# Aqasch/TensorRL-QAS

Measured on AMD Instinct MI355X. Metric: VQE env-steps/sec, higher is better.
Workload: dtype f64

## Files before the change

### tensorrl-qas_amd/csrc/vqe_device.h

```cpp
#pragma once
#include <hip/hip_runtime.h>
#include <stdint.h>
#ifdef VQE_STAMPS
__device__ unsigned long long g_cby_dbg[8];
__device__ unsigned long long g_cby_in_out[2];
__device__ long long g_cby_t0_unused;
#if defined(__HIP_DEVICE_COMPILE__)
#define CBY_STAMP_RESET() long long cby_t0_ = (long long)__builtin_readcyclecounter(); (void)cby_t0_
#define CBY_STAMP(k)                                                                               \
  {                                                                                                \
    const long long t_ = (long long)__builtin_readcyclecounter();                                  \
    if (ctx.tid == 0 && Ctx::nth > 1) __hip_atomic_fetch_add(&g_cby_dbg[k], (unsigned long long)(t_ - cby_t0_), __ATOMIC_RELAXED, __HIP_MEMORY_SCOPE_AGENT); \
    cby_t0_ = (long long)__builtin_readcyclecounter();                                             \
  }
#else
#define CBY_STAMP_RESET()
#define CBY_STAMP(k)
#endif
#endif
#include "cobyla_m0.h"
#include "vqe_geo.h"

namespace vqe {

// ... 451 lines not shown
            L.ops[nops] = Op{xm[r.q0], zm[r.q0], r.pidx, r.kind | (int)(((c >> r.q0) & 1u) << 8)};
          ++nops;
          break;
        default: break;
      }
    }
    int permuted = (c != 0);
    for (int q = 0; q < n; ++q) if (xm[q] != (1u << q)) permuted = 1;
    L.meta[0] = nops < A.max_ops ? nops : A.max_ops;
    L.meta[1] = (int32_t)c;
    L.meta[2] = phase;
    L.meta[3] = permuted;
    L.meta[6] = permuted;
    L.meta[7] = (int32_t)c;
  }
  __syncthreads();
}

template <int N>
__device__ __forceinline__ void patch_noise_wave(const BatchArgs& A, int b, uint64_t eval_id, const Lds& L, int skip,
                                                 bool canonical, int lane, int skip_end) {
  const int G = A.gate_count[b];
  const int4* gsrc = (const int4*)(A.gates + A.gate_begin[b]);
  {
    Op* exe = N >= 10 ? L.sched : L.ops;
    const int kmax = L.meta[0];
    const uint64_t lt_mask = lane ? (~0ull >> (64 - lane)) : 0ull;
    const uint64_t nkey = noise_key(A.noise.seed, (uint64_t)b, eval_id);
    uint32_t c = 0;
    int ny = 0, kbase = 0;
    int4 rnext = lane < G ? gsrc[lane] : make_int4(-1, 0, 0, 0);
    for (int base = 0; base < G; base += 64) {
      const int i = base + lane;
      int kind = -1, q0 = 0, q1 = 0, code = 0;
      const int4 r = rnext;
      if (i + 64 < G) rnext = gsrc[i + 64];
      if (i < G && !(i >= skip && i < skip_end)) {
        kind = r.x; q0 = r.y; q1 = r.z < 0 ? 0 : r.z;
        if (kind == G_DEPOL1 || kind == G_DEPOL2) {
          const double u = noise_uniform_k(nkey, (uint64_t)(i - ((skip >= 0 && i >= skip_end) ? skip_end - skip : 0)));
          if (kind == G_DEPOL1) { if (u < A.noise.p1) code = 1 + (int)(u / A.noise.p1 * 3.0); }
          else if (u < A.noise.p2) code = 1 + (int)(u / A.noise.p2 * 15.0);
        }
      }
      const int pa = kind == G_DEPOL1 ? code : (kind == G_DEPOL2 ? (code & 3) : 0);
      const int pb = kind == G_DEPOL2 ? (code >> 2) : 0;
      const uint32_t flip_a = (pa == 1 || pa == 2) ? 1u << q0 : 0u;
      const uint32_t flip_b = (pb == 1 || pb == 2) ? 1u << q1 : 0u;
      const uint32_t cnot_m = kind == G_CNOT ? 1u << q1 : 0u;
      const int nrec = (kind >= G_RX && kind <= G_DEPOL1) ? 1 : (kind == G_DEPOL2 ? 2 : 0);
      const uint32_t w1 = flip_a | ((uint32_t)q0 << 16) | ((uint32_t)q1 << 24);
      const uint32_t w2 = cnot_m | (flip_b << 16);
      const uint64_t has1 = __ballot(nrec >= 1), has2 = __ballot(nrec == 2);
      const int k0 = kbase + __popcll(has1 & lt_mask) + __popcll(has2 & lt_mask);
      kbase += __popcll(has1) + __popcll(has2);
      ny += __popcll(__ballot(pa == 2)) + __popcll(__ballot(pb == 2));
      uint64_t inv0 = 0, inv1 = 0;
      const int cnt = G - base < 64 ? G - base : 64;
      int j0 = 0;
      if (c == 0) {
        const uint64_t flips = __ballot((flip_a | flip_b) != 0u);
        j0 = flips ? __ffsll((long long)flips) - 1 : cnt;
      }
      for (int j = j0; j < cnt; ++j) {
        const uint32_t a = (uint32_t)__builtin_amdgcn_readlane((int)w1, j);
        const uint32_t bw = (uint32_t)__builtin_amdgcn_readlane((int)w2, j);
        c ^= a & 0xffffu;
        const uint32_t b0 = (c >> ((a >> 16) & 31u)) & 1u;
        c ^= (0u - b0) & (bw & 0xffffu);
        inv0 |= (uint64_t)b0 << j;
        c ^= bw >> 16;
        inv1 |= (uint64_t)((c >> (a >> 24)) & 1u) << j;
      }
      auto apply = [&](int pk, int sign, int pauli) {
        if (pk < kmax) {
          Op* o = exe + L.sidx[pk];
          int kd = o->kind;
          if (pauli >= 0) kd = (kd & ~0xff) | ((pauli == 2 || pauli == 3) ? OP_PZ : OP_NOP);
          o->kind = (kd & ~0x100) | (sign << 8);
        }
      };
      if (nrec >= 1) apply(k0, (int)((inv0 >> lane) & 1ull), kind <= G_RZ ? -1 : pa);
      if (nrec == 2) apply(k0 + 1, (int)((inv1 >> lane) & 1ull), pb);
    }
    {
      const int ns = N >= 10 ? L.meta[4] : kmax;
      int lead = 0;
      for (int base = ((ns - 1) / 64) * 64; base >= 0; base -= 64) {
        const int k = base + lane;
        const int kd = k < ns ? exe[k].kind : 0;
        const bool nop = k < ns && (kd & 0xff) == OP_NOP;
        const uint64_t m = __ballot(nop);
        const uint64_t behind = lane < 63 ? (m >> (lane + 1)) : 0ull;
        const int in_chunk = 63 - lane;
        int run = behind == ~0ull >> (lane + 1) && lane < 63 ? in_chunk : (lane < 63 ? __ffsll((long long)~behind) - 1 : 0);
        if (run >= in_chunk) run = in_chunk + lead;
        if (k < ns) exe[k].kind = (kd & 0x00ffffff) | ((run < 255 ? run : 255) << 24);
        lead = (m == ~0ull) ? 64 + lead : __ffsll((long long)~m) - 1;
      }
    }
    if (lane == 0) {
      uint32_t cs = c;
      if (N >= 10 && canonical) {
        cs = 0;
        for (int q = 0; q < N; ++q) cs |= (uint32_t)parity32(A.ham.mrow[q] & c) << q;
      }
      L.meta[1] = (int32_t)cs;
      L.meta[2] = (3 * ny) & 3;
      L.meta[3] = L.meta[6] | (c != 0);
      L.meta[7] = (int32_t)c;
    }
  }
}

template <int N>
__device__ __forceinline__ void patch_noise(const BatchArgs& A, int b, uint64_t eval_id, const Lds& L, int skip,
                                            bool canonical, int skip_end = 0) {
  if (threadIdx.x < 64) patch_noise_wave<N>(A, b, eval_id, L, skip, canonical, (int)threadIdx.x, skip_end);
  __syncthreads();
}

}
#include "vqe_reg.h"
namespace vqe {

template <int N>
__device__ __forceinline__ void compile_all(const BatchArgs& A, int b, uint64_t eval_id, const Lds& L, int skip = -1,
                                            bool canonical = true, bool slots = false, int skip_end = 0) {
  compile_ops(A, b, eval_id, L, skip, slots, skip_end);
  if constexpr (N < 10) {
    if (slots) {
      for (int k = threadIdx.x; k < L.meta[0]; k += (int)blockDim.x) L.sidx[k] = (uint16_t)k;
      __syncthreads();
    }
  }
  if constexpr (N >= kRegMinQubits) {
    if (threadIdx.x == 0) schedule_ops<N>(L);
    __syncthreads();
    if (canonical) {
      uint32_t zrow = 0, cbit = 0;
      if (threadIdx.x < N) {
        const uint32_t m = A.ham.mrow[threadIdx.x];
        for (int q = 0; q < N; ++q) if ((m >> q) & 1u) zrow ^= L.zm[q];
        cbit = (uint32_t)parity32(m & (uint32_t)L.meta[1]) << threadIdx.x;
      }
      uint32_t cnew = cbit;
#pragma unroll
      for (int o = 8; o > 0; o >>= 1) cnew |= __shfl_xor(cnew, o, 16);
      __syncthreads();
      if (threadIdx.x < N) L.zm[threadIdx.x] = zrow;
      if (threadIdx.x == 0) L.meta[1] = (int32_t)cnew;
      __syncthreads();
    }
  }
}

template <int N, bool SLOTS = true>
__device__ __forceinline__ void run_ops(const Lds& L, const double* theta, int P, int p_hole = -1) {
  constexpr int kThreads = Geo<N>::NT;
  constexpr uint32_t DIM = 1u << N;
  constexpr int NP = (DIM / 2 + kThreads - 1) / kThreads;
  constexpr int NA = (DIM + kThreads - 1) / kThreads;
  const int tid = threadIdx.x;
  for (int j = tid; j < P; j += kThreads) {
    if (j == p_hole) continue;
    double s, c;
    sincos(0.5 * theta[j - (p_hole >= 0 && j > p_hole)], &s, &c);
    L.cs[j] = make_double2(c, s);
  }
  __syncthreads();
  const int nops = L.meta[0];
  for (int o = 0; o < nops; ++o) {
    const Op op = L.ops[o];
    const int kind = op.kind & 0xff;
    if constexpr (SLOTS) o += (int)((uint32_t)op.kind >> 24);
    if (kind == OP_NOP) continue;
    const int inv = (op.kind >> 8) & 1;
    if (kind == OP_RX || kind == OP_RY) {
      const double2 cs = L.cs[op.pidx];
      const int hb = 31 - __clz((int)op.xm);
      if (kind == OP_RX) {
#pragma unroll
        for (int k = 0; k < NP; ++k) {
          const uint32_t q = tid + k * kThreads;
          if (DIM / 2 >= kThreads || q < DIM / 2) {
            const uint32_t p0 = insert0(q, hb), p1 = p0 ^ op.xm;
            const double2 a0 = L.psi[p0], a1 = L.psi[p1];
            L.psi[p0] = make_double2(cs.x * a0.x - cs.y * a1.y, cs.x * a0.y + cs.y * a1.x);
            L.psi[p1] = make_double2(cs.x * a1.x - cs.y * a0.y, cs.x * a1.y + cs.y * a0.x);
          }
        }
      } else {
#pragma unroll
        for (int k = 0; k < NP; ++k) {
          const uint32_t q = tid + k * kThreads;
          if (DIM / 2 >= kThreads || q < DIM / 2) {
            const uint32_t p0 = insert0(q, hb), p1 = p0 ^ op.xm;
            const double s0 = (parity32(p0 & op.zm) ^ inv) ? -cs.y : cs.y;
            const double2 a0 = L.psi[p0], a1 = L.psi[p1];
            L.psi[p0] = make_double2(cs.x * a0.x + s0 * a1.x, cs.x * a0.y + s0 * a1.y);
            L.psi[p1] = make_double2(cs.x * a1.x - s0 * a0.x, cs.x * a1.y - s0 * a0.y);
          }
        }
      }
    } else if (kind == OP_RZ) {
      const double2 cs = L.cs[op.pidx];
#pragma unroll
      for (int k = 0; k < NA; ++k) {
        const uint32_t p = tid + k * kThreads;
        if (DIM >= kThreads || p < DIM) {
          const double s = (parity32(p & op.zm) ^ inv) ? -cs.y : cs.y;
          const double2 a = L.psi[p];
          L.psi[p] = make_double2(cs.x * a.x - s * a.y, cs.x * a.y + s * a.x);
        }
      }
    } else if (kind == OP_PZ) {
#pragma unroll
      for (int k = 0; k < NA; ++k) {
        const uint32_t p = tid + k * kThreads;
        if ((DIM >= kThreads || p < DIM) && (parity32(p & op.zm) ^ inv)) {
          const double2 a = L.psi[p];
          L.psi[p] = make_double2(-a.x, -a.y);
        }
      }
    }
    __syncthreads();
  }
  if (L.meta[3]) {
    const uint32_t c = (uint32_t)L.meta[1];
    double2 tmp[NA];
#pragma unroll
    for (int k = 0; k < NA; ++k) {
      const uint32_t i = tid + k * kThreads;
      if (DIM >= kThreads || i < DIM) {
        uint32_t v = i ^ c, p = 0;
#pragma unroll
        for (int q = 0; q < N; ++q) p ^= ((v >> q) & 1u) ? L.xm[q] : 0u;
        tmp[k] = L.psi[p];
      }
    }
    __syncthreads();
#pragma unroll
    for (int k = 0; k < NA; ++k) {
      const uint32_t i = tid + k * kThreads;
      if (DIM >= kThreads || i < DIM) L.psi[i] = tmp[k];
    }
    __syncthreads();
  }
}

template <int N>
__device__ __forceinline__ void load_init(const Lds& L, const double2* init) {
  constexpr int kThreads = Geo<N>::NT;
  constexpr uint32_t DIM = 1u << N;
  constexpr int NA = (DIM + kThreads - 1) / kThreads;
#pragma unroll
  for (int k = 0; k < NA; ++k) {
    const uint32_t p = threadIdx.x + k * kThreads;
    if (DIM >= kThreads || p < DIM) L.psi[p] = init[p];
  }
}


constexpr int kEnergyBatch = 4;

#define VQE_ENERGY_PAIRS(X, HB, DEXPR)                                                             \
  {                                                                                                \
    const uint32_t base = insert0(tid, (HB)) << 4, basex = base ^ ((X) << 4);                     \
    uint32_t kbit[KB > 0 ? KB : 1];                                                                \
    _Pragma("unroll") for (int i = 0; i < KB; ++i)                                                \
      kbit[i] = 16u << (LT + i + ((LT + i) >= (HB) ? 1 : 0));                                     \
    double p0s = 0.0, p1s = 0.0;                                                                   \
    _Pragma("unroll") for (int k0 = 0; k0 < NP; k0 += kEnergyBatch) {                             \
      constexpr int NB = NP < kEnergyBatch ? NP : kEnergyBatch;                                   \
      double2 pa[NB], pb[NB];                                                                      \
      _Pragma("unroll") for (int kk = 0; kk < NB; ++kk) {                                         \
        const int k = k0 + kk;                                                                     \
        uint32_t kc = 0;                                                                           \
        _Pragma("unroll") for (int i = 0; i < KB; ++i) if ((k >> i) & 1) kc ^= kbit[i];           \
        const bool live = FULL || tid + (uint32_t)k * kThreads < DIM / 2;                         \
        pb[kk] = live ? *(const double2*)(psi_b + (base ^ kc)) : make_double2(0.0, 0.0);         \
        pa[kk] = live ? *(const double2*)(psi_b + (basex ^ kc)) : make_double2(0.0, 0.0);        \
      }                                                                                            \
      __builtin_amdgcn_sched_barrier(0);                                                           \
      _Pragma("unroll") for (int kk = 0; kk < NB; ++kk) {                                         \
        const int k = k0 + kk;                                                                     \
        const double v = (pa[kk].x * pb[kk].x + pa[kk].y * pb[kk].y) * (DEXPR);                   \
        if (k & 1) p1s += v; else p0s += v;                                                       \
      }                                                                                            \
    }                                                                                              \
    acc0 += p0s;                                                         \
    acc1 += p1s;                                                                                   \
  }

#define VQE_ENERGY_CONSUME(G, D)                                                                   \
  {                                                                                                \
    const GroupMeta m = L.gm[G];                                                                   \
    const uint32_t x = (uint32_t)__builtin_amdgcn_readfirstlane((int)m.x);                        \
    const int hb = __builtin_amdgcn_readfirstlane(m.hb);                                          \
    VQE_ENERGY_PAIRS(x, hb, D[k])                                                                  \
  }

template <int N>
__device__ __forceinline__ void energy_real_lds(const Lds& L, const double* __restrict__ tables, int g0, int g1,
                                                double& acc0, double& acc1) {
  constexpr int kThreads = Geo<N>::NT;
// ... 524 lines not shown
        first += kStage * kThreads;
      }
    }
    for (int i0 = first; i0 < nw; i0 += kStage * kThreads) {
      double2 v[kStage];
#pragma unroll
      for (int k = 0; k < kStage; ++k) {
        const int i = i0 + k * kThreads;
        v[k] = s[i < nw ? i : nw - 1];
      }
#pragma unroll
      for (int k = 0; k < kStage; ++k) asm volatile("" : "+v"(v[k].x), "+v"(v[k].y));
#pragma unroll
      for (int k = 0; k < kStage; ++k) {
        const int i = i0 + k * kThreads;
        if (i < nw) d[i] = v[k];
      }
    }
    __syncthreads();
  }
  __device__ __forceinline__ bool out(bool full = true, double2* cs_out = nullptr, int P = 0, int p_hole = -1) {
    if (threadIdx.x == 0) { pub[0] = want; pub[1] = nfvals; }
    __syncthreads();
    want = pub[0]; nfvals = pub[1];
    if (!staged || resident) return false;
    const bool light = VQE_LIGHT_OUT && !full && want && cs_out != nullptr;
    if (light) {
      for (int j = threadIdx.x; j < P; j += kThreads) {
        if (j == p_hole) continue;
        double sn, cn;
        sincos(0.5 * lmem[j - (p_hole >= 0 && j > p_hole)], &sn, &cn);
        cs_out[j] = make_double2(cn, sn);
      }
    }
    const double2* s = (const double2*)lmem;
    double2* d = (double2*)gmem;
    const int nw = (words + 1) / 2;
    for (int i0 = threadIdx.x; i0 < nw; i0 += kStage * kThreads) {
      double2 v[kStage];
#pragma unroll
      for (int k = 0; k < kStage; ++k) {
        const int i = i0 + k * kThreads;
        v[k] = s[i < nw ? i : nw - 1];
      }
#pragma unroll
      for (int k = 0; k < kStage; ++k) asm volatile("" : "+v"(v[k].x), "+v"(v[k].y));
#pragma unroll
      for (int k = 0; k < kStage; ++k) {
        const int i = i0 + k * kThreads;
        if (i < nw) d[i] = v[k];
      }
    }
    if (light) {
      asm volatile("s_waitcnt lgkmcnt(0)\n\ts_barrier" ::: "memory");
      return true;
    }
    __syncthreads();
    return false;
  }
  template <bool FIRST, class Cob, class Ptr>
  __device__ __forceinline__ void call(Ptr mem, double f, double rhobeg, double rhoend, int maxfun) {
    Cob cob;
    cob.ctx.tid = Cob::P == 0 ? 0 : (int)(threadIdx.x % (unsigned)decltype(cob.ctx)::nth);
    if constexpr (!std::is_base_of<WaveCtx, decltype(cob.ctx)>::value) cob.ctx.red = red;
    if constexpr (decltype(cob.ctx)::kTile) {
      if constexpr (std::is_base_of<WaveCtx, decltype(cob.ctx)>::value) {
        cob.ctx.tile = (lds_double*)tile;
        cob.ctx.shared = (lds_double*)tile + Cob::kTileDoubles;
      } else {
        cob.ctx.tile = (lds_double*)lmem + (threadIdx.x >> 6) * Cob::kTileDoubles;
        cob.ctx.shared = (lds_double*)lmem + (kThreads / 64) * Cob::kTileDoubles;
      }
    }
    int nn = n;
    if constexpr (N >= 10) asm volatile("" : "+s"(mem), "+s"(nn));
    cob.bind(mem, nn);
    if (FIRST) {
      want = cob.start(rhobeg, rhoend, maxfun);
    } else {
      cob.load_state();
      want = cob.tell(f);
    }
    nfvals = cob.nfvals;
    cob.save_state();
  }
  bool cs_ready;
  template <bool FIRST, class Side>
  __device__ __forceinline__ int run(double f, double rhobeg, double rhoend, int maxfun, Side side, bool full = true,
                                     double2* cs_out = nullptr, int P = 0, int p_hole = -1) {
#ifdef VQE_STAMPS
    const long long t0 = clock64();
#endif
    in();
#ifdef VQE_STAMPS
    const long long t1 = clock64();
#endif
    if (kBlock && block) {
      if constexpr (kBlock) {
        if (kThreads == 64 || (threadIdx.x >= 64 && threadIdx.x < 128)) side();
        call<FIRST, CobB>(gmem, f, rhobeg, rhoend, maxfun);
      }
    } else if (threadIdx.x < 64) {
      if (staged) call<FIRST, CobL>((lds_double*)lmem, f, rhobeg, rhoend, maxfun);
      else if (rows_ctx()) {
        if constexpr (kRowsG) call<FIRST, CobR>(gmem, f, rhobeg, rhoend, maxfun);
      } else call<FIRST, CobG>(gmem, f, rhobeg, rhoend, maxfun);
      if constexpr (kThreads == 64) side();
    } else if (threadIdx.x < 128) {
#ifdef VQE_STAMPS
      const long long ts0 = clock64();
#endif
      side();
#ifdef VQE_STAMPS
      if (threadIdx.x == 64 && !FIRST) atomicAdd(&g_cby_dbg[6], (unsigned long long)(clock64() - ts0));
#endif
    }
#ifdef VQE_STAMPS
    const long long t2 = clock64();
#endif
    cs_ready = out(full, cs_out, P, p_hole);
#ifdef VQE_STAMPS
    if (threadIdx.x == 0 && !FIRST) {
      atomicAdd(&g_cby_dbg[7], (unsigned long long)(t2 - t1));
      atomicAdd(&g_cby_in_out[0], (unsigned long long)(t1 - t0));
      atomicAdd(&g_cby_in_out[1], (unsigned long long)(clock64() - t2));
    }
#endif
    return want;
  }
  __device__ __forceinline__ int start(double rhobeg, double rhoend, int maxfun, bool full = true, double2* cs_out = nullptr,
                                       int P = 0, int p_hole = -1) {
    return run<true>(0.0, rhobeg, rhoend, maxfun, NoSide(), full, cs_out, P, p_hole);
  }
  template <class Side>
  __device__ __forceinline__ int tell(double f, unsigned long long* __restrict__ dbg, Side side, bool full = true,
                                      double2* cs_out = nullptr, int P = 0, int p_hole = -1) {
#ifdef VQE_STAMPS
    const long long t0 = clock64();
#endif
    const int w = run<false>(f, 0.0, 0.0, 0, side, full, cs_out, P, p_hole);
#ifdef VQE_STAMPS
    if (threadIdx.x == 0) atomicAdd(dbg + 4, (unsigned long long)(clock64() - t0));
#endif
    return w;
  }
};

template <int N>
__global__ void __launch_bounds__(Geo<N>::NT) k_lds_energy(BatchArgs A) {
  extern __shared__ __attribute__((aligned(16))) unsigned char smem[];
  const Lds L = carve(smem, N, A.max_ops, A.max_params, A.ham.n_groups, A.max_pair);
  const int b = blockIdx.x;
  const bool noisy = (A.noise.p1 > 0.0 || A.noise.p2 > 0.0);
  stage_groups(A.ham, L);
  if constexpr (N >= 10) stage_cls<N>(A.ham, L);
  compile_all<N>(A, b, 0, L, -1, true, noisy);
  if (noisy) patch_noise<N>(A, b, A.noise.eval_base, L, -1, true);
  double e = lds_evaluate<N, true>(A, L, A.theta + A.par_begin[b], A.par_count[b]);
  if (A.noise.shot_sigma != 0.0) e += A.noise.shot_sigma * noise_gauss(A.noise.seed, (uint64_t)b, A.noise.eval_base);
  if (threadIdx.x == 0) { A.fout[b] = e; if (A.nfev) A.nfev[b] = 1; }
}

template <int N>
__global__ void __launch_bounds__(Geo<N>::NT) k_lds_state(BatchArgs A) {
  constexpr int kThreads = Geo<N>::NT;
  extern __shared__ __attribute__((aligned(16))) unsigned char smem[];
  const Lds L = carve(smem, N, A.max_ops, A.max_params, A.ham.n_groups, A.max_pair);
  const bool noisy_state = (A.noise.p1 > 0.0 || A.noise.p2 > 0.0);
  compile_all<N>(A, 0, 0, L, -1, false, noisy_state);
  if (noisy_state) patch_noise<N>(A, 0, A.noise.eval_base, L, -1, false);
  if constexpr (N >= kRegMinQubits) {
    run_ops_reg<N, true>(L, A.init, A.theta + A.par_begin[0], A.par_count[0]);
  } else {
    load_init<N>(L, A.init);
    __syncthreads();
    run_ops<N>(L, A.theta + A.par_begin[0], A.par_count[0]);
  }
  const int ph = L.meta[2];
  for (uint32_t p = threadIdx.x; p < (1u << N); p += kThreads) {
    double2 a = L.psi[p];
    if (ph == 1) a = make_double2(-a.y, a.x);
    else if (ph == 2) a = make_double2(-a.x, -a.y);
    else if (ph == 3) a = make_double2(a.y, -a.x);
    A.state_out[p] = a;
  }
}

template <int N, bool WIDE = (N >= 10 && Geo<N>::NT >= 256), bool NOISY = false>
__global__ void __launch_bounds__(Geo<N>::NT, Geo<N>::WPS) k_lds_minimize(BatchArgs A) {
  constexpr int kThreads = Geo<N>::NT;
  extern __shared__ __attribute__((aligned(16))) unsigned char smem[];
  const Lds L = carve(smem, N, A.max_ops, A.max_params, A.ham.n_groups, A.max_pair);
  const int b = A.order[blockIdx.x];
  const int P = A.par_count[b];
  const double* theta = A.theta + A.par_begin[b];
  double* xout = A.xout + A.par_begin[b];
  constexpr bool noisy = NOISY;
  const int skip = A.new_gate ? A.new_gate[b] : -1;
  int p_hole = -1;
  int skip_end = skip + 1;
  if (skip >= 0) {
    const GateRec r = A.gates[A.gate_begin[b] + skip];
    if (r.kind >= G_RX && r.kind <= G_RZ) p_hole = r.pidx;
    if (skip + 1 < A.gate_count[b]) {
      const GateRec f = A.gates[A.gate_begin[b] + skip + 1];
      if ((f.kind == G_DEPOL1 && r.kind >= G_RX && r.kind <= G_RZ && f.q0 == r.q0) ||
          (f.kind == G_DEPOL2 && r.kind == G_CNOT && f.q0 == r.q0 && f.q1 == r.q1))
        skip_end = skip + 2;
    }
  }
  const int Popt = P - (p_hole >= 0);
  stage_groups(A.ham, L);
  if constexpr (N >= 10) stage_cls<N>(A.ham, L);
  StagedCobyla<N, WIDE> sc;
  sc.cs_ready = false;
  const bool full_out = N < 10 || A.trace != nullptr;
  int phase = 0, nfev = 1;
  bool need_compile = true;
  bool patched = false;
  double fret = 0.0, flast = 0.0;
  if (Popt > 0) {
    sc.init(A.scratch + A.scratch_begin[b], L, Popt);
    for (int j = threadIdx.x; j < P; j += kThreads)
      if (j != p_hole) sc.x()[j - (p_hole >= 0 && j > p_hole)] = theta[j];
    __syncthreads();
    sc.start(A.rhobeg, A.rhoend, A.maxfun, full_out, L.cs, P, p_hole);
    phase = 1;
  }
  for (;;) {
    const double* th = phase == 0 ? theta : (phase == 1 ? sc.x() : xout);
    const int sk = phase == 2 ? -1 : skip;
    const int ske = phase == 2 ? 0 : skip_end;
    const int ph = phase == 2 ? -1 : p_hole;
    const uint64_t eid = A.noise.eval_base +
                         (phase == 1 ? (uint64_t)sc.nfvals : (phase == 2 ? (uint64_t)A.maxfun + 1 : 0));
    if (need_compile) { compile_all<N>(A, b, 0, L, sk, true, noisy, ske); need_compile = false; patched = false; }
    if (noisy && !patched) patch_noise<N>(A, b, eid, L, sk, true, ske);
    patched = false;
    const bool csr = phase == 1 && sc.cs_ready;
    double e = lds_evaluate<N, NOISY>(A, L, th, P, ph, [&]() { if (phase == 1) sc.prefetch(); }, csr);
    if (A.noise.shot_sigma != 0.0) e += A.noise.shot_sigma * noise_gauss(A.noise.seed, (uint64_t)b, eid);
    bool finished_opt = false;
    if (phase == 0) {
      fret = e;
      for (int j = threadIdx.x; j < P; j += kThreads) {
        xout[j] = A.env_step ? (double)(float)theta[j] : theta[j];
        A.xraw[A.par_begin[b] + j] = theta[j];
      }
      finished_opt = true;
    } else if (phase == 1) {
      flast = e;
      if (A.trace) {
        double* tr = A.trace + ((size_t)b * A.maxfun + (size_t)(sc.nfvals - 1)) * (size_t)(1 + A.max_params);
        if (threadIdx.x == 0) tr[0] = e;
        for (int j = threadIdx.x; j < Popt; j += kThreads) tr[1 + j] = sc.x()[j];
      }
#ifdef VQE_STAMPS
      const long long tt0 = clock64();
#endif
      const uint64_t eid_next = A.noise.eval_base + (uint64_t)sc.nfvals + 1;
      const int want = sc.tell(e, A.dbg, [&]() {
        if (noisy) patch_noise_wave<N>(A, b, eid_next, L, sk, true, (int)(threadIdx.x & 63), ske);
      }, full_out, L.cs, P, p_hole);
      patched = noisy && want;
#ifdef VQE_STAMPS
      if (threadIdx.x == 0) atomicAdd(A.dbg + 3, (unsigned long long)(clock64() - tt0));
#endif
      if (!want) {
        for (int j = threadIdx.x; j < P; j += kThreads) {
          const double v = (j == p_hole) ? theta[j] : sc.x()[j - (p_hole >= 0 && j > p_hole)];
          xout[j] = A.env_step ? (double)(float)v : v;
          A.xraw[A.par_begin[b] + j] = v;
        }
        const double* st = sc.state();
        fret = ((int)st[11] == cby::DONE_RHOEND && (int)st[10] == 1) ? flast : st[4];
        nfev = sc.nfvals;
        finished_opt = true;
      }
    } else {
      fret = e;
      break;
    }
    if (finished_opt) {
      if (!A.env_step) break;
      __syncthreads();
      phase = 2;
      need_compile = true;
    }
  }
  if (threadIdx.x == 0) { A.fout[b] = fret; A.nfev[b] = nfev; }
}

}
```

### tensorrl-qas_amd/csrc/vqe_reg.h

```cpp
#pragma once
#include "vqe_geo.h"

namespace vqe {

enum : int { OP_RELAYOUT = 5 };

struct LayoutRec {
  uint32_t e[5];
  uint32_t pos;
  uint32_t pos8;
  uint32_t pad;
};

struct Basis {
  uint32_t* e;
  int32_t* piv;
  int k;
  __device__ void clear() { k = 0; }
  __device__ uint32_t reduce(uint32_t v) const {
    for (int i = 0; i < k; ++i) if ((v >> piv[i]) & 1u) v ^= e[i];
    return v;
  }
  __device__ bool add(uint32_t v) {
    v = reduce(v);
    if (!v) return false;
    const int p = 31 - __clz((int)v);
    for (int i = 0; i < k; ++i) if ((e[i] >> p) & 1u) e[i] ^= v;
    e[k] = v; piv[k] = p; ++k;
    return true;
  }
  __device__ uint32_t coords(uint32_t v) const {
    uint32_t j = 0;
    for (int i = 0; i < k; ++i) j |= ((v >> piv[i]) & 1u) << i;
    return j;
  }
};

template <int N>
__device__ __forceinline__ void emit_layout(const Basis& B, LayoutRec* out) {
  uint32_t pivmask = 0;
  for (int i = 0; i < 5; ++i) out->e[i] = i < B.k ? B.e[i] : 0u;
  for (int i = 0; i < B.k; ++i) pivmask |= 1u << B.piv[i];
  uint32_t pos = 0, pos8 = 0;
  int cnt = 0;
  for (int b = 0; b < N; ++b)
    if (!((pivmask >> b) & 1u)) {
      if (cnt < 8) pos |= (uint32_t)b << (4 * cnt); else pos8 = (uint32_t)b;
      ++cnt;
    }
  out->pos = pos;
  out->pos8 = pos8;
}

template <int R>
__device__ __forceinline__ uint32_t sign_word(uint32_t svec) {
  constexpr uint32_t pat[5] = {0xAAAAAAAAu, 0xCCCCCCCCu, 0xF0F0F0F0u, 0xFF00FF00u, 0xFFFF0000u};
  uint32_t w = 0;
#pragma unroll
  for (int i = 0; i < R; ++i) if ((svec >> i) & 1u) w ^= pat[i];
  return w;
}

template <int N>
__device__ __forceinline__ void schedule_ops(const Lds& L) {
  constexpr int R = N - Geo<N>::LT;
  const int nraw = L.meta[0];
  int ns = 0, nl = 0;
  Basis B;
  B.e = (uint32_t*)L.sb;
  B.piv = (int32_t*)L.sb + 8;
  auto open_layout = [&](int from) {
    B.clear();
    for (int k = from; k < nraw && B.k < R; ++k) {
      const int kd = L.ops[k].kind & 0xff;
      if (kd == OP_RX || kd == OP_RY) B.add(L.ops[k].xm);
    }
    for (int b = N - 1; b >= 0 && B.k < R; --b) B.add(1u << b);
    emit_layout<N>(B, &L.lay[nl]);
    ++nl;
  };
  open_layout(0);
  for (int o = 0; o < nraw; ++o) {
    const Op op = L.ops[o];
    const int kd = op.kind & 0xff;
    uint32_t j = 0;
    if (kd == OP_RX || kd == OP_RY) {
      if (B.reduce(op.xm) != 0) {
        open_layout(o);
        L.sched[ns++] = Op{(uint32_t)(nl - 1), 0u, -1, OP_RELAYOUT};
      }
      j = B.coords(op.xm);
    }
    uint32_t svec = 0;
    for (int i = 0; i < R; ++i) svec |= (uint32_t)parity32(op.zm & B.e[i]) << i;
    L.sidx[o] = (uint16_t)ns;
    L.sched[ns++] = Op{sign_word<R>(svec), op.zm, op.pidx >= 0 ? op.pidx * 16 : 0, op.kind | (int32_t)(j << 16)};
  }
  L.sched[ns] = Op{0u, 0u, 0, 0};
  L.meta[4] = ns;
  L.meta[5] = nl;
}

template <int LT>
__device__ __forceinline__ uint32_t deposit(uint32_t tid, uint32_t pos, uint32_t pos8) {
  uint32_t b = 0;
#pragma unroll
  for (int j = 0; j < 8; ++j) b |= ((tid >> j) & 1u) << ((pos >> (4 * j)) & 15u);
  if (LT > 8) b |= ((tid >> 8) & 1u) << pos8;
  return b;
}

template <int R>
__device__ __forceinline__ uint32_t combo(const uint32_t (&e)[5], int r) {
  uint32_t v = 0;
#pragma unroll
  for (int i = 0; i < R; ++i) if ((r >> i) & 1) v ^= e[i];
  return v;
}

__device__ __forceinline__ double flip_if(double v, uint32_t w, int r) {
  const uint32_t hi = (uint32_t)__double2hiint(v) ^ (((w >> r) & 1u) << 31);
  return __hiloint2double((int)hi, __double2loint(v));
}

__device__ __forceinline__ void rot2x2(double& x0, double& y0, double& x1, double& y1, double c, double s0,
                                       double s1) {
  double t0, t1;
  asm("v_mul_f64 %4, %7, %1\n\t"
      "v_mul_f64 %5, %8, %3\n\t"
      "v_mul_f64 %1, %6, %1\n\t"
      "v_mul_f64 %3, %6, %3\n\t"
      "v_fmac_f64 %1, %7, %0\n\t"
      "v_fmac_f64 %3, %8, %2\n\t"
      "v_fma_f64 %0, %6, %0, -%4\n\t"
      "v_fma_f64 %2, %6, %2, -%5"
      : "+v"(x0), "+v"(y0), "+v"(x1), "+v"(y1), "=&v"(t0), "=&v"(t1)
      : "v"(c), "v"(s0), "v"(s1));
}

template <int NA, int J>
__device__ __forceinline__ void rx_pairs(double2 (&amp)[NA], double c, double s) {
  static_assert(J > 0 && J < NA, "partner mask out of range");
  constexpr int HB = 31 - __builtin_clz(J);
#pragma unroll
  for (int r = 0; r < NA; ++r) {
    if ((r >> HB) & 1) continue;
    const int r2 = r ^ J;
    rot2x2(amp[r].x, amp[r2].y, amp[r2].x, amp[r].y, c, s, s);
  }
}

template <int NA, int J>
__device__ __forceinline__ void ry_pairs(double2 (&amp)[NA], double c, double s, uint32_t w) {
  constexpr int HB = 31 - __builtin_clz(J);
#pragma unroll
  for (int r = 0; r < NA; ++r) {
    if ((r >> HB) & 1) continue;
    const int r2 = r ^ J;
    const double s0 = flip_if(s, w, r);
    rot2x2(amp[r2].x, amp[r].x, amp[r2].y, amp[r].y, c, s0, s0);
  }
}

#define VQE_PAIR_CASE(J, CALL) case J: if constexpr (J < NA) { CALL; } break;
#define VQE_PAIR_SWITCH(j, F, ...)                                                                 \
  switch (j) {                                                                                     \
    VQE_PAIR_CASE(1, (F<NA, 1>(__VA_ARGS__))) VQE_PAIR_CASE(2, (F<NA, 2>(__VA_ARGS__)))            \
    VQE_PAIR_CASE(3, (F<NA, 3>(__VA_ARGS__))) VQE_PAIR_CASE(4, (F<NA, 4>(__VA_ARGS__)))            \
    VQE_PAIR_CASE(5, (F<NA, 5>(__VA_ARGS__))) VQE_PAIR_CASE(6, (F<NA, 6>(__VA_ARGS__)))            \
    VQE_PAIR_CASE(7, (F<NA, 7>(__VA_ARGS__))) VQE_PAIR_CASE(8, (F<NA, 8>(__VA_ARGS__)))            \
    VQE_PAIR_CASE(9, (F<NA, 9>(__VA_ARGS__))) VQE_PAIR_CASE(10, (F<NA, 10>(__VA_ARGS__)))          \
    VQE_PAIR_CASE(11, (F<NA, 11>(__VA_ARGS__))) VQE_PAIR_CASE(12, (F<NA, 12>(__VA_ARGS__)))        \
    VQE_PAIR_CASE(13, (F<NA, 13>(__VA_ARGS__))) VQE_PAIR_CASE(14, (F<NA, 14>(__VA_ARGS__)))        \
    VQE_PAIR_CASE(15, (F<NA, 15>(__VA_ARGS__))) VQE_PAIR_CASE(16, (F<NA, 16>(__VA_ARGS__)))        \
    VQE_PAIR_CASE(17, (F<NA, 17>(__VA_ARGS__))) VQE_PAIR_CASE(18, (F<NA, 18>(__VA_ARGS__)))        \
    VQE_PAIR_CASE(19, (F<NA, 19>(__VA_ARGS__))) VQE_PAIR_CASE(20, (F<NA, 20>(__VA_ARGS__)))        \
    VQE_PAIR_CASE(21, (F<NA, 21>(__VA_ARGS__))) VQE_PAIR_CASE(22, (F<NA, 22>(__VA_ARGS__)))        \
    VQE_PAIR_CASE(23, (F<NA, 23>(__VA_ARGS__))) VQE_PAIR_CASE(24, (F<NA, 24>(__VA_ARGS__)))        \
    VQE_PAIR_CASE(25, (F<NA, 25>(__VA_ARGS__))) VQE_PAIR_CASE(26, (F<NA, 26>(__VA_ARGS__)))        \
    VQE_PAIR_CASE(27, (F<NA, 27>(__VA_ARGS__))) VQE_PAIR_CASE(28, (F<NA, 28>(__VA_ARGS__)))        \
    VQE_PAIR_CASE(29, (F<NA, 29>(__VA_ARGS__))) VQE_PAIR_CASE(30, (F<NA, 30>(__VA_ARGS__)))        \
    VQE_PAIR_CASE(31, (F<NA, 31>(__VA_ARGS__)))                                                    \
    default: break;                                                                                \
  }

template <int N, bool SLOTS = false>
__device__ __forceinline__ void run_ops_reg(const Lds& L, const double2* __restrict__ init, const double* theta, int P,
                                   int p_hole = -1, unsigned long long* __restrict__ dbg = nullptr, bool cs_ready = false) {
#ifdef VQE_STAMPS
  const long long ts0 = clock64();
  long long trel = 0;
#endif
  constexpr int kThreads = Geo<N>::NT;
  constexpr int LT = Geo<N>::LT;
  constexpr int R = N - LT;
  constexpr int NA = 1 << R;
  int tid = threadIdx.x;
  asm volatile("" : "+v"(tid));
  if (!cs_ready) {
    for (int j = tid; j < P; j += kThreads) {
      if (j == p_hole) continue;
      double s, c;
      sincos(0.5 * theta[j - (p_hole >= 0 && j > p_hole)], &s, &c);
      L.cs[j] = make_double2(c, s);
    }
  }
  double2 amp[NA];
  uint32_t e[5];
  typedef __attribute__((address_space(3))) unsigned char lds_byte;
  lds_byte* psi_l = (lds_byte*)L.psi;
  auto lds_get = [&](uint32_t off) {
    const d2v_t v = *(const __attribute__((address_space(3))) d2v_t*)(psi_l + off);
    return make_double2(v.x, v.y);
  };
  auto lds_put = [&](uint32_t off, const double2& a) {
    d2v_t v; v.x = a.x; v.y = a.y;
    *(__attribute__((address_space(3))) d2v_t*)(psi_l + off) = v;
  };
  uint32_t base = deposit<LT>(tid, L.lay[0].pos, L.lay[0].pos8);
  {
    const LayoutRec lr = L.lay[0];
#pragma unroll
    for (int i = 0; i < 5; ++i) e[i] = lr.e[i] << 4;
    const unsigned char* init_b = (const unsigned char*)init;
#pragma unroll
    for (int r = 0; r < NA; ++r) amp[r] = *(const double2*)(init_b + ((base << 4) ^ combo<R>(e, r)));
  }
  __builtin_amdgcn_s_waitcnt(0x0F70);
  __syncthreads();
  const int nops = L.meta[4];
#ifdef VQE_STAMPS
  const long long ts1 = clock64();
#endif
  const unsigned char* cs_b = (const unsigned char*)L.cs;
  Op nxt = L.sched[0];
  double2 ncs = *(const double2*)(cs_b + nxt.pidx);
  for (int o = 0; o < nops; ++o) {
    const Op op = nxt;
    const double2 cs = ncs;
    if constexpr (SLOTS) o += (int)((uint32_t)__builtin_amdgcn_readfirstlane(op.kind) >> 24);
    nxt = L.sched[o + 1];
    ncs = *(const double2*)(cs_b + nxt.pidx);
    const int kind = op.kind & 0xff;
    if (kind == OP_RELAYOUT) {
#ifdef VQE_STAMPS
      const long long tr0 = clock64();
#endif
      __syncthreads();
      {
        const uint32_t b16 = base << 4;
#pragma unroll
        for (int r = 0; r < NA; ++r) lds_put(b16 ^ combo<R>(e, r), amp[r]);
      }
      const LayoutRec lr = L.lay[op.xm];
#pragma unroll
      for (int i = 0; i < 5; ++i) e[i] = lr.e[i] << 4;
      base = deposit<LT>(tid, lr.pos, lr.pos8);
      __syncthreads();
      {
        const uint32_t b16 = base << 4;
#pragma unroll
        for (int r = 0; r < NA; ++r) amp[r] = lds_get(b16 ^ combo<R>(e, r));
      }
#ifdef VQE_STAMPS
      trel += clock64() - tr0;
#endif
      continue;
    }
    if (kind == OP_NOP) continue;
    const int inv = (op.kind >> 8) & 1;
    const uint32_t flip = (uint32_t)(parity32(op.zm & base) ^ inv);
    const uint32_t w = op.xm ^ (0u - flip);
    const int jm = (op.kind >> 16) & 0xff;
    if (kind == OP_RX) {
      VQE_PAIR_SWITCH(jm, rx_pairs, amp, cs.x, cs.y)
    } else if (kind == OP_RY) {
      VQE_PAIR_SWITCH(jm, ry_pairs, amp, cs.x, cs.y, w)
    } else if (kind == OP_RZ) {
#pragma unroll
      for (int r = 0; r < NA; r += 2)
        rot2x2(amp[r].x, amp[r].y, amp[r + 1].x, amp[r + 1].y, cs.x, flip_if(cs.y, w, r), flip_if(cs.y, w, r + 1));
    } else if (kind == OP_PZ) {
#pragma unroll
      for (int r = 0; r < NA; ++r) amp[r] = make_double2(flip_if(amp[r].x, w, r), flip_if(amp[r].y, w, r));
    }
  }
#ifdef VQE_STAMPS
  const long long ts2 = clock64();
#endif
  uint32_t ib = (uint32_t)L.meta[1] << 4;
  uint32_t ae[5] = {0u, 0u, 0u, 0u, 0u};
#pragma unroll
  for (int q = 0; q < N; ++q) {
    const uint32_t z = L.zm[q];
    ib ^= (uint32_t)parity32(z & base) << (q + 4);
#pragma unroll
    for (int i = 0; i < R; ++i) ae[i] |= (uint32_t)parity32(z & (e[i] >> 4)) << (q + 4);
  }
  __syncthreads();
#pragma unroll
  for (int r = 0; r < NA; ++r) lds_put(ib ^ combo<R>(ae, r), amp[r]);
  __syncthreads();
#ifdef VQE_STAMPS
  if (threadIdx.x == 0 && dbg) {
    atomicAdd(dbg + 5, (unsigned long long)(ts1 - ts0));
    atomicAdd(dbg + 6, (unsigned long long)trel);
    atomicAdd(dbg + 7, (unsigned long long)(clock64() - ts2));
  }
#endif
}

}
```

Measured before the change: 13370.

## Precompute final scatter tables and replace bit deposit with pivot-spread addressing

Moves the per-thread final-writeback parity computation (looping over all qubits for base and each register direction) into a one-time table built after scheduling. Thread addresses are split into low/high nibble lookups and XORed. Layout records now store pre-shifted directions and pivot positions, so the per-thread base comes from an add-based spread instead of an 8–9 step deposit. Layout fields are made wave-uniform with readfirstlane, and absolute LDS addresses are used. In exchange it adds an alignment requirement on psi, and kernels return NaN when psi is misaligned. The scatter tables also reuse parts of the zm, xm and sb buffers.

```diff
diff --git a/tensorrl-qas_amd/csrc/vqe_device.h b/tensorrl-qas_amd/csrc/vqe_device.h
--- a/tensorrl-qas_amd/csrc/vqe_device.h
+++ b/tensorrl-qas_amd/csrc/vqe_device.h
@@ -627,6 +627,8 @@
       if (threadIdx.x == 0) L.meta[1] = (int32_t)cnew;
       __syncthreads();
     }
+    hoist_scatter<N>(L);
+    __syncthreads();
   }
 }
 
@@ -1457,6 +1459,10 @@
   const Lds L = carve(smem, N, A.max_ops, A.max_params, A.ham.n_groups, A.max_pair);
   const int b = blockIdx.x;
   const bool noisy = (A.noise.p1 > 0.0 || A.noise.p2 > 0.0);
+  if (!psi_aligned<N>(L)) {
+    if (threadIdx.x == 0) { A.fout[b] = __builtin_nan(""); if (A.nfev) A.nfev[b] = 0; }
+    return;
+  }
   stage_groups(A.ham, L);
   if constexpr (N >= 10) stage_cls<N>(A.ham, L);
   compile_all<N>(A, b, 0, L, -1, true, noisy);
@@ -1472,6 +1478,10 @@
   extern __shared__ __attribute__((aligned(16))) unsigned char smem[];
   const Lds L = carve(smem, N, A.max_ops, A.max_params, A.ham.n_groups, A.max_pair);
   const bool noisy_state = (A.noise.p1 > 0.0 || A.noise.p2 > 0.0);
+  if (!psi_aligned<N>(L)) {
+    for (uint32_t p = threadIdx.x; p < (1u << N); p += kThreads) A.state_out[p] = make_double2(__builtin_nan(""), __builtin_nan(""));
+    return;
+  }
   compile_all<N>(A, 0, 0, L, -1, false, noisy_state);
   if (noisy_state) patch_noise<N>(A, 0, A.noise.eval_base, L, -1, false);
   if constexpr (N >= kRegMinQubits) {
@@ -1515,6 +1525,10 @@
     }
   }
   const int Popt = P - (p_hole >= 0);
+  if (!psi_aligned<N>(L)) {
+    if (threadIdx.x == 0) { A.fout[b] = __builtin_nan(""); A.nfev[b] = 0; }
+    return;
+  }
   stage_groups(A.ham, L);
   if constexpr (N >= 10) stage_cls<N>(A.ham, L);
   StagedCobyla<N, WIDE> sc;
diff --git a/tensorrl-qas_amd/csrc/vqe_reg.h b/tensorrl-qas_amd/csrc/vqe_reg.h
--- a/tensorrl-qas_amd/csrc/vqe_reg.h
+++ b/tensorrl-qas_amd/csrc/vqe_reg.h
@@ -6,10 +6,9 @@
 enum : int { OP_RELAYOUT = 5 };
 
 struct LayoutRec {
-  uint32_t e[5];
-  uint32_t pos;
-  uint32_t pos8;
-  uint32_t pad;
+  uint32_t e16[4];
+  uint32_t piv;
+  uint32_t pad[3];
 };
 
 struct Basis {
@@ -38,18 +37,15 @@
 
 template <int N>
 __device__ __forceinline__ void emit_layout(const Basis& B, LayoutRec* out) {
+  static_assert(N - Geo<N>::LT <= 4, "LayoutRec holds four register directions");
   uint32_t pivmask = 0;
-  for (int i = 0; i < 5; ++i) out->e[i] = i < B.k ? B.e[i] : 0u;
+  for (int i = 0; i < 4; ++i) out->e16[i] = i < B.k ? B.e[i] << 4 : 0u;
   for (int i = 0; i < B.k; ++i) pivmask |= 1u << B.piv[i];
-  uint32_t pos = 0, pos8 = 0;
+  uint32_t piv = 0;
   int cnt = 0;
   for (int b = 0; b < N; ++b)
-    if (!((pivmask >> b) & 1u)) {
-      if (cnt < 8) pos |= (uint32_t)b << (4 * cnt); else pos8 = (uint32_t)b;
-      ++cnt;
-    }
-  out->pos = pos;
-  out->pos8 = pos8;
+    if ((pivmask >> b) & 1u) piv |= (uint32_t)b << (4 * cnt++);
+  out->piv = piv;
 }
 
 template <int R>
@@ -101,17 +97,39 @@
   L.meta[5] = nl;
 }
 
-template <int LT>
-__device__ __forceinline__ uint32_t deposit(uint32_t tid, uint32_t pos, uint32_t pos8) {
-  uint32_t b = 0;
-#pragma unroll
-  for (int j = 0; j < 8; ++j) b |= ((tid >> j) & 1u) << ((pos >> (4 * j)) & 15u);
-  if (LT > 8) b |= ((tid >> 8) & 1u) << pos8;
-  return b;
-}
-
 template <int R>
-__device__ __forceinline__ uint32_t combo(const uint32_t (&e)[5], int r) {
+__device__ __forceinline__ uint32_t spread(uint32_t t, uint32_t piv) {
+#pragma unroll
+  for (int i = 0; i < R; ++i) t += t & (~0u << ((piv >> (4 * i)) & 15u));
+  return t;
+}
+
+__device__ __forceinline__ uint32_t* scatter_lo(const Lds& L) { return L.zm + 16; }
+__device__ __forceinline__ uint32_t* scatter_hi(const Lds& L) { return L.xm; }
+__device__ __forceinline__ uint32_t* scatter_ae(const Lds& L) { return L.sb; }
+
+template <int N>
+__device__ __forceinline__ void hoist_scatter(const Lds& L) {
+  constexpr int LT = Geo<N>::LT;
+  constexpr int R = N - LT;
+  constexpr uint32_t NHI = 1u << (LT - 4);
+  static_assert(LT >= 4 && NHI <= 32 && N <= 16, "scatter tables live in L.xm and the upper half of L.zm");
+  const LayoutRec* lr = (const LayoutRec*)L.lay + (L.meta[5] - 1);
+  const uint32_t t = threadIdx.x;
+  if (t < 16u + NHI + (uint32_t)R) {
+    uint32_t p;
+    uint32_t* dst;
+    if (t < 16u) { p = spread<R>(t, lr->piv); dst = scatter_lo(L) + t; }
+    else if (t < 16u + NHI) { p = spread<R>((t - 16u) << 4, lr->piv); dst = scatter_hi(L) + (t - 16u); }
+    else { p = lr->e16[t - 16u - NHI] >> 4; dst = scatter_ae(L) + (t - 16u - NHI); }
+    uint32_t v = 0;
+    for (int q = 0; q < N; ++q) v |= (uint32_t)parity32(L.zm[q] & p) << (q + 4);
+    *dst = v;
+  }
+}
+
+template <int R>
+__device__ __forceinline__ uint32_t combo(const uint32_t (&e)[4], int r) {
   uint32_t v = 0;
 #pragma unroll
   for (int i = 0; i < R; ++i) if ((r >> i) & 1) v ^= e[i];
@@ -184,6 +202,12 @@
     default: break;                                                                                \
   }
 
+template <int N>
+__device__ __forceinline__ bool psi_aligned(const Lds& L) {
+  typedef __attribute__((address_space(3))) unsigned char lds_byte;
+  return N < kRegMinQubits || ((uint32_t)(uintptr_t)(lds_byte*)L.psi & ((16u << N) - 1u)) == 0u;
+}
+
 template <int N, bool SLOTS = false>
 __device__ __forceinline__ void run_ops_reg(const Lds& L, const double2* __restrict__ init, const double* theta, int P,
                                    int p_hole = -1, unsigned long long* __restrict__ dbg = nullptr, bool cs_ready = false) {
@@ -206,22 +230,25 @@
     }
   }
   double2 amp[NA];
-  uint32_t e[5];
+  uint32_t e[4] = {0u, 0u, 0u, 0u};
+  uint32_t base;
+  auto enter_layout = [&](const LayoutRec* lr) {
+#pragma unroll
+    for (int i = 0; i < R; ++i) e[i] = (uint32_t)__builtin_amdgcn_readfirstlane((int)lr->e16[i]);
+    base = spread<R>((uint32_t)tid, (uint32_t)__builtin_amdgcn_readfirstlane((int)lr->piv));
+  };
   typedef __attribute__((address_space(3))) unsigned char lds_byte;
-  lds_byte* psi_l = (lds_byte*)L.psi;
-  auto lds_get = [&](uint32_t off) {
-    const d2v_t v = *(const __attribute__((address_space(3))) d2v_t*)(psi_l + off);
+  const uint32_t psi_a = (uint32_t)(uintptr_t)(lds_byte*)L.psi;
+  auto lds_get = [&](uint32_t addr) {
+    const d2v_t v = *(const __attribute__((address_space(3))) d2v_t*)(uintptr_t)addr;
     return make_double2(v.x, v.y);
   };
-  auto lds_put = [&](uint32_t off, const double2& a) {
+  auto lds_put = [&](uint32_t addr, const double2& a) {
     d2v_t v; v.x = a.x; v.y = a.y;
-    *(__attribute__((address_space(3))) d2v_t*)(psi_l + off) = v;
+    *(__attribute__((address_space(3))) d2v_t*)(uintptr_t)addr = v;
   };
-  uint32_t base = deposit<LT>(tid, L.lay[0].pos, L.lay[0].pos8);
+  enter_layout(L.lay);
   {
-    const LayoutRec lr = L.lay[0];
-#pragma unroll
-    for (int i = 0; i < 5; ++i) e[i] = lr.e[i] << 4;
     const unsigned char* init_b = (const unsigned char*)init;
 #pragma unroll
     for (int r = 0; r < NA; ++r) amp[r] = *(const double2*)(init_b + ((base << 4) ^ combo<R>(e, r)));
@@ -248,17 +275,14 @@
 #endif
       __syncthreads();
       {
-        const uint32_t b16 = base << 4;
+        const uint32_t b16 = (base << 4) + psi_a;
 #pragma unroll
         for (int r = 0; r < NA; ++r) lds_put(b16 ^ combo<R>(e, r), amp[r]);
       }
-      const LayoutRec lr = L.lay[op.xm];
-#pragma unroll
-      for (int i = 0; i < 5; ++i) e[i] = lr.e[i] << 4;
-      base = deposit<LT>(tid, lr.pos, lr.pos8);
+      enter_layout(L.lay + op.xm);
       __syncthreads();
       {
-        const uint32_t b16 = base << 4;
+        const uint32_t b16 = (base << 4) + psi_a;
 #pragma unroll
         for (int r = 0; r < NA; ++r) amp[r] = lds_get(b16 ^ combo<R>(e, r));
       }
@@ -288,15 +312,10 @@
 #ifdef VQE_STAMPS
   const long long ts2 = clock64();
 #endif
-  uint32_t ib = (uint32_t)L.meta[1] << 4;
-  uint32_t ae[5] = {0u, 0u, 0u, 0u, 0u};
-#pragma unroll
-  for (int q = 0; q < N; ++q) {
-    const uint32_t z = L.zm[q];
-    ib ^= (uint32_t)parity32(z & base) << (q + 4);
-#pragma unroll
-    for (int i = 0; i < R; ++i) ae[i] |= (uint32_t)parity32(z & (e[i] >> 4)) << (q + 4);
-  }
+  const uint32_t ib = (((uint32_t)L.meta[1] << 4) ^ scatter_lo(L)[tid & 15] ^ scatter_hi(L)[tid >> 4]) + psi_a;
+  uint32_t ae[4] = {0u, 0u, 0u, 0u};
+#pragma unroll
+  for (int i = 0; i < R; ++i) ae[i] = (uint32_t)__builtin_amdgcn_readfirstlane((int)scatter_ae(L)[i]);
   __syncthreads();
 #pragma unroll
   for (int r = 0; r < NA; ++r) lds_put(ib ^ combo<R>(ae, r), amp[r]);
```

New measurement: 13580, median of 6. +1.5%, better.
